# qiqiqicheng/news-recommendation-tc

Hardware: AMD Instinct MI355X
Metric: recalled pairs/sec (YouTubeDNN top-30) + DIN scored pairs/sec, 1/2/4/8 MI355X (higher is better)
Workload: dtype fp16

## Files before the change

### include/nrk.h

```cpp
#ifndef NRK_H
#define NRK_H

#include <stddef.h>
#include <stdint.h>

#ifdef __cplusplus
extern "C" {
#endif

typedef void* nrk_stream_t;

#define NRK_OK 0
#define NRK_EINVAL 1
#define NRK_EHIP 2
#define NRK_EUNSUPPORTED 3

const char* nrk_last_error(void);
#define NRK_ABI_VERSION 3
int nrk_abi_version(void);


int nrk_tt_user_fwd(const float* user_table, int64_t n_user_rows, const float* item_table,
                    int64_t n_item_rows, int dim, const int32_t* uid, const int32_t* hist,
                    const int32_t* hist_len, int64_t n, int seq_len, const float* w0,
                    const float* b0, int h0, const float* w1, const float* b1, int h1,
                    float* out, nrk_stream_t stream);

int nrk_tt_user_fwd_layers(const float* user_table, int64_t n_user_rows, const float* item_table,
                           int64_t n_item_rows, int dim, const int32_t* uid, const int32_t* hist,
                           const int32_t* hist_len, int64_t n, int seq_len, const float* weights, int n_layers,
                           const int* widths, float* out, nrk_stream_t stream);
int nrk_tt_item_fwd(const float* item_table, int64_t n_item_rows, int dim, const int32_t* ids,
                    int64_t n, float* out, nrk_stream_t stream);


size_t nrk_tt_train_workspace_bytes(int64_t n_user_rows, int64_t n_item_rows, int dim, int n_layers,
                                    const int* widths, int seq_len, int batch);

int nrk_tt_train_grad(const float* user_table, int64_t n_user_rows, const float* item_table,
                      int64_t n_item_rows, int dim, const float* weights, int n_layers, const int* widths,
                      const int64_t* log_off, const int32_t* log_items, const int32_t* s_user,
                      const int32_t* s_pos, const int32_t* s_target, const float* s_label, int batch,
                      int seq_len, float p, uint64_t seed, int64_t step, float* loss, float* w_grad,
                      int32_t* u_rows, float* u_vals, int32_t* u_count, int32_t* i_rows, float* i_vals,
                      int32_t* i_count, void* workspace, size_t workspace_bytes, nrk_stream_t stream);

int nrk_tt_dropout_mask(uint64_t seed, int64_t step, int layer, int batch, int width, float p, float* out,
                        nrk_stream_t stream);

int nrk_tt_adam_step(float* weights, float* w_m, float* w_v, const float* w_grad, int64_t n_weights,
                     float* user_table, float* u_m, float* u_v, int64_t n_user_rows, const int32_t* u_rows,
                     const float* u_vals, const int32_t* u_count, float* item_table, float* i_m, float* i_v,
                     int64_t n_item_rows, const int32_t* i_rows, const float* i_vals, const int32_t* i_count,
                     int dim, double lr, double beta1, double beta2, double eps, int64_t t,
                     nrk_stream_t stream);

int nrk_tt_make_samples_count(const int64_t* log_off, int64_t n_users, int64_t* pos_off, nrk_stream_t stream);
int nrk_tt_make_samples(const int64_t* log_off, const int32_t* log_items, int64_t n_users,
                        const int64_t* pos_off, int64_t n_pos, int negsample, const int32_t* pool,
                        int64_t n_pool, uint64_t seed, int32_t* s_user, int32_t* s_pos, int32_t* s_target,
                        float* s_label, nrk_stream_t stream);


size_t nrk_ip_catalog_bytes(int64_t n_items, int dim);
int nrk_ip_catalog_build(const float* items, int64_t n_items, int dim, void* catalog,
                         nrk_stream_t stream);

size_t nrk_ip_topk_workspace_bytes(int64_t n_users, int64_t n_items, int dim, int k);
int nrk_ip_topk(const float* users, int64_t n_users, const float* items, const void* catalog,
                int64_t n_items, int dim, int k, int64_t row_offset, float* out_scores,
                int32_t* out_rows, double* out_exact, void* workspace, size_t workspace_bytes,
                nrk_stream_t stream);

int nrk_ip_topk_screen(const float* users, int64_t n_users, const void* catalog, int64_t n_items,
                       int dim, int k, void* workspace, size_t workspace_bytes,
                       nrk_stream_t stream);
int nrk_ip_topk_scan(const float* users, int64_t n_users, const void* catalog, int64_t n_items, int dim, int k,
                     void* workspace, size_t workspace_bytes, nrk_stream_t stream);
int nrk_ip_topk_select(const float* users, int64_t n_users, const void* catalog, int64_t n_items, int dim, int k,
                       void* workspace, size_t workspace_bytes, nrk_stream_t stream);
int nrk_ip_topk_finish(const float* users, int64_t n_users, const float* items,
                       const void* catalog, int64_t n_items,
                       int dim, int k, int64_t row_offset, float* out_scores, int32_t* out_rows,
                       double* out_exact, void* workspace, size_t workspace_bytes,
                       nrk_stream_t stream);

int nrk_ip_topk_bound(const float* users, int64_t n_users, const void* catalog, int64_t n_items, int dim,
                      int k, int m, float* out_bound, void* workspace, size_t workspace_bytes,
                      nrk_stream_t stream);
int nrk_ip_topk_apply_bound(int64_t n_users, const float* bounds, int n_lists, int m, int k, void* workspace,
                            size_t workspace_bytes, nrk_stream_t stream);

int nrk_ip_topk_tile_blocks(int dim);

int nrk_ip_topk_shard_screen(const float* users, int64_t n_users, const void* catalog, int64_t n_items, int dim,
                             int k, int64_t blk_lo, int64_t blk_hi, int m, float* out_bound, void* workspace,
                             size_t workspace_bytes, nrk_stream_t stream);
int nrk_ip_topk_shard_band(int64_t n_users, int64_t n_items, int dim, int k, const float* bounds, int n_lists,
                           int m, int x_cap, void* workspace, size_t workspace_bytes, void* out_ent,
                           int32_t* out_cnt, nrk_stream_t stream);
int nrk_ip_topk_refine_x(const float* users, int64_t n_users, const float* items, const void* catalog,
                         int64_t n_items, int dim, int k, int64_t row_offset, const void* band, int n_src,
                         int64_t src_users, int x_cap, const int32_t* src_cnt, const float* ucut,
                         const int32_t* ovf_in, float* out_scores, int32_t* out_rows, double* out_exact,
                         void* workspace, size_t workspace_bytes, nrk_stream_t stream);

int nrk_topk_merge(const double* in_exact, const int32_t* in_rows, int n_lists,
                   int64_t list_stride, int64_t n_users, int k_in, int k_out, float* out_scores,
                   int32_t* out_rows, double* out_exact, nrk_stream_t stream);

#define NRK_IP_QUERY_MAX_USERS 4096
size_t nrk_ip_query_workspace_bytes(int64_t n_users, int64_t n_items, int dim, int k);
int nrk_ip_query_plan(int64_t n_users, int64_t n_items, int dim, int k, int32_t out[4]);
int nrk_ip_query(const float* users, int64_t n_users, const float* items, int64_t n_items, int dim, int k,
                 int64_t row_offset, float* out_scores, int32_t* out_rows, double* out_exact, void* workspace,
                 size_t workspace_bytes, nrk_stream_t stream);


int nrk_row_normalize(const float* x, int64_t n, int dim, float* out, float* norms,
                      nrk_stream_t stream);


int nrk_itemcf_pair_offsets(const int64_t* offsets, int64_t n_users, int64_t* pair_off,
                            nrk_stream_t stream);
size_t nrk_itemcf_workspace_bytes(int64_t n_pairs, int32_t n_items);
int nrk_itemcf_sim(const int64_t* offsets, int64_t n_users, const int32_t* items,
                   const int64_t* ts, const double* created, int32_t n_items,
                   const int64_t* pair_off, int64_t n_pairs, double loc_alpha,
                   double loc_alpha_rev, double loc_beta, double time_alpha,
                   double created_alpha, int32_t* out_i, int32_t* out_j, double* out_v,
                   int64_t* out_first, int64_t* out_n, int64_t* out_cnt, void* workspace,
                   size_t workspace_bytes, nrk_stream_t stream);

int nrk_itemcf_topn(const int64_t* row_off, int64_t n_rows, const int32_t* cols,
                    const double* vals, const int64_t* first, int topn, int32_t* out_cols,
                    double* out_vals, int32_t* out_cnt, nrk_stream_t stream);

int nrk_itemcf_pairs(const int64_t* offsets, int64_t n_users, const int32_t* items, const int64_t* ts,
                     const double* created, int32_t n_items, const int64_t* pair_off, int64_t slot_base,
                     double loc_alpha, double loc_alpha_rev, double loc_beta, double time_alpha,
                     double created_alpha, uint64_t* keys, int32_t* slots, double* w, int64_t* item_cnt,
                     nrk_stream_t stream);
size_t nrk_itemcf_reduce_workspace_bytes(int64_t n);
int nrk_itemcf_reduce(const uint64_t* keys, const int32_t* slots, const double* w, int64_t n, int32_t n_items,
                      const int64_t* item_cnt, int32_t* out_i, int32_t* out_j, double* out_v,
                      int64_t* out_first, int64_t* out_n, void* workspace, size_t workspace_bytes,
                      nrk_stream_t stream);

int nrk_itemcf_row_offsets(const int32_t* ei, int64_t n, int64_t n_rows, int64_t* row_off,
                           nrk_stream_t stream);

int nrk_itemcf_recall_offsets(const int64_t* q_slot, int64_t n_query, const int64_t* offsets,
                              const int32_t* items, const int32_t* nbr_cnt, int64_t* cand_off,
                              nrk_stream_t stream);
size_t nrk_itemcf_recall_workspace_bytes(int64_t n_cand);
int nrk_itemcf_recall(const int64_t* q_slot, int64_t n_query, const int64_t* offsets, const int32_t* items,
                      const int32_t* nbr_cols, const double* nbr_vals, const int32_t* nbr_cnt, int topn,
                      const double* created, int32_t n_items, const int32_t* hot, int n_hot,
                      const int32_t* emb_cols, const double* emb_vals, const int32_t* emb_cnt, int ke,
                      double loc_beta, double created_alpha, const int64_t* cand_off, int64_t n_cand,
                      int topk, int32_t* out_items, double* out_scores, int32_t* out_src,
                      int32_t* out_cnt, void* workspace, size_t workspace_bytes, nrk_stream_t stream);


size_t nrk_usercf_workspace_bytes(int64_t n_users, int64_t n_clicks, int topn);
int nrk_usercf_topn(const int64_t* i_off, int32_t n_items, const int32_t* i_users, const int64_t* u_off,
                    int64_t n_users, const int32_t* u_items, int64_t n_clicks, const double* act, const double* pen,
                    int topn, int32_t* out_cols, double* out_vals, int64_t* out_cnt, int32_t* out_nnz,
                    void* workspace, size_t workspace_bytes, nrk_stream_t stream);
int nrk_usercf_sim(const int64_t* i_off, int32_t n_items, const int32_t* i_users, const int64_t* u_off,
                   int64_t n_users, const int32_t* u_items, int64_t n_clicks, const double* act, const double* pen,
                   const int64_t* row_off, int64_t n_entries, int32_t* out_v, double* out_s, int64_t* out_first,
                   void* workspace, size_t workspace_bytes, nrk_stream_t stream);

int nrk_usercf_recall_offsets(const int64_t* q_slot, int64_t n_query, const int64_t* offsets,
                              const int32_t* nbr_cols, const int32_t* nbr_cnt, int topn, int64_t* cand_off,
                              nrk_stream_t stream);
size_t nrk_usercf_recall_workspace_bytes(int64_t n_cand);
int nrk_usercf_recall(const int64_t* q_slot, int64_t n_query, const int64_t* offsets, const int32_t* items,
// ... 184 lines not shown
```

### news-recommendation-tc_amd/csrc/tower.hip

```cpp
#include "tower_common.h"

namespace nrk {

template <int D>
__global__ __launch_bounds__(256) __attribute__((amdgpu_waves_per_eu(4))) void tt_user_kernel(
    const float* __restrict__ user_table, const float* __restrict__ item_table,
    const int32_t* __restrict__ uid, const int32_t* __restrict__ hist,
    const int32_t* __restrict__ hist_len, int64_t n, int T, const float* __restrict__ w0,
    const float* __restrict__ b0, int h0, const float* __restrict__ w1,
    const float* __restrict__ b1, int h1, float* __restrict__ out) {
    static_assert(D % 2 == 0 && D >= 16 && D <= 64 && (D & (D - 1)) == 0, "tt_user_kernel: D in {16, 32, 64}");
    extern __shared__ __attribute__((aligned(16))) float lds[];
    const int S0 = 2 * D + 4, h0p = (h0 + 3) & ~3, S1 = h0p + 4, h1p = (h1 + 3) & ~3;
    float* sw0 = lds;
    float* sb0 = sw0 + h0 * S0;
    float* sw1 = sb0 + h0p;
    float* sb1 = sw1 + h1 * S1;
    float* sx = sb1 + h1p + (threadIdx.x >> 6) * (2 * D + 128);
    for (int i = threadIdx.x; i < h0 * 2 * D; i += blockDim.x) sw0[(i / (2 * D)) * S0 + i % (2 * D)] = w0[i];
    for (int i = threadIdx.x; i < h0; i += blockDim.x) sb0[i] = b0[i];
    for (int i = threadIdx.x; i < h1 * h0; i += blockDim.x) sw1[(i / h0) * S1 + i % h0] = w1[i];
    for (int i = threadIdx.x; i < h1; i += blockDim.x) sb1[i] = b1[i];
    __syncthreads();

    constexpr int P = WAVE / D;
    constexpr int CH = 8;
    const int lane = threadIdx.x & 63, wave = threadIdx.x >> 6;
    const int d = lane % D, ph = lane / D;
    const int64_t wstride = (int64_t)gridDim.x * 4;
    auto meta = [&](int64_t uu, int& len, int32_t& uidv, int32_t& hv) {
        const bool ok = uu < n;
        len = ok ? hist_len[uu] : 0;
        uidv = ok ? uid[uu] : 0;
        hv = ok && lane < T ? hist[uu * T + lane] : 0;
    };
    int64_t u = (int64_t)blockIdx.x * 4 + wave;
    int len, uidv;
    int32_t hv;
    meta(u, len, uidv, hv);
    float pout = 0.0f;
    int64_t pu = -1;
    for (; u < n; u += wstride) {
        int nlen, nuid;
        int32_t nhv;
        meta(u + wstride, nlen, nuid, nhv);
        const float xu = user_table[(int64_t)uidv * D + d];
        float sum = 0.0f;
        const int nit = (len + P - 1) / P;
        for (int i0 = 0; i0 < nit; i0 += CH) {
            float v[CH];
#pragma unroll
            for (int e = 0; e < CH; ++e) {
                const int t = ph + P * (i0 + e);
                const int32_t r = __shfl(hv, t < T ? t : 0, WAVE);
                v[e] = item_table[(int64_t)(t < len ? r : 0) * D + d];
            }
            if (i0 == 0 && pu >= 0) {
                if (lane < h1) out[pu * h1 + lane] = pout;
                pu = -1;
            }
#pragma unroll
            for (int e = 0; e < CH; ++e)
                if (ph + P * (i0 + e) < len) sum += v[e];
        }
#pragma unroll
        for (int off = D; off < WAVE; off <<= 1) sum += __shfl_xor(sum, off, WAVE);
        const float xm = sum / ((float)len + 1e-8f);
        if (lane < D) {
            sx[lane] = xu;
            sx[D + lane] = xm;
        }
        __builtin_amdgcn_wave_barrier();
        float y0 = 0.0f, y1 = 0.0f;
        {
#pragma clang fp contract(off)
            float z0 = lane < h0 ? sb0[lane] : 0.0f;
            float z1 = lane + WAVE < h0 ? sb0[lane + WAVE] : 0.0f;
            const float* wr0 = sw0 + (lane < h0 ? lane : 0) * S0;
            const float* wr1 = sw0 + (lane + WAVE < h0 ? lane + WAVE : 0) * S0;
            if (h0 > WAVE) {
#pragma unroll 2
                for (int q = 0; q < 2 * D; q += 4) {
                    const float4 xq = *reinterpret_cast<const float4*>(sx + q);
                    const float4 a = *reinterpret_cast<const float4*>(wr0 + q);
                    const float4 b = *reinterpret_cast<const float4*>(wr1 + q);
                    z0 += a.x * xq.x;
                    z0 += a.y * xq.y;
                    z0 += a.z * xq.z;
                    z0 += a.w * xq.w;
                    z1 += b.x * xq.x;
                    z1 += b.y * xq.y;
                    z1 += b.z * xq.z;
                    z1 += b.w * xq.w;
                }
            } else {
#pragma unroll 2
                for (int q = 0; q < 2 * D; q += 4) {
                    const float4 xq = *reinterpret_cast<const float4*>(sx + q);
                    const float4 a = *reinterpret_cast<const float4*>(wr0 + q);
                    z0 += a.x * xq.x;
                    z0 += a.y * xq.y;
                    z0 += a.z * xq.z;
                    z0 += a.w * xq.w;
                }
            }
            y0 = fmaxf(z0, 0.0f);
            y1 = fmaxf(z1, 0.0f);
        }
        float* sy = sx + 2 * D;
        if (lane < h0) sy[lane] = y0;
        if (lane + WAVE < h0) sy[lane + WAVE] = y1;
        __builtin_amdgcn_wave_barrier();
        float v = 0.0f;
        {
#pragma clang fp contract(off)
            float z = lane < h1 ? sb1[lane] : 0.0f;
            const float* wr = sw1 + (lane < h1 ? lane : 0) * S1;
            int q = 0;
            for (; q + 4 <= h0; q += 4) {
                const float4 yq = *reinterpret_cast<const float4*>(sy + q);
                const float4 a = *reinterpret_cast<const float4*>(wr + q);
                z += a.x * yq.x;
                z += a.y * yq.y;
                z += a.z * yq.z;
                z += a.w * yq.w;
            }
            for (; q < h0; ++q) z += wr[q] * sy[q];
            v = lane < h1 ? fmaxf(z, 0.0f) : 0.0f;
        }
        __builtin_amdgcn_wave_barrier();
        const float nn = sqrtf(wave_sum_f32(v * v));
        v = v / fmaxf(nn, 1e-12f);
        float n2 = sqrtf(wave_sum_f32(v * v));
        if (n2 == 0.0f) n2 = 1.0f;
        if (pu >= 0 && lane < h1) out[pu * h1 + lane] = pout;
        pout = v / n2;
        pu = u;
        len = nlen;
        uidv = nuid;
        hv = nhv;
    }
    if (pu >= 0 && lane < h1) out[pu * h1 + lane] = pout;
}

template <int D>
__global__ __launch_bounds__(256) void tt_user_mlp_kernel(
    const float* __restrict__ user_table, const float* __restrict__ item_table,
    const int32_t* __restrict__ uid, const int32_t* __restrict__ hist,
    const int32_t* __restrict__ hist_len, int64_t n, int T, const float* __restrict__ wts, TtLayers ly,
    float* __restrict__ out) {
    __shared__ float sx[4][2][TT_MAXW > 2 * D ? TT_MAXW : 2 * D];
    const int lane = threadIdx.x & 63, wave = threadIdx.x >> 6;
    const int64_t wstride = (int64_t)gridDim.x * 4;
    for (int64_t u = (int64_t)blockIdx.x * 4 + wave; u < n; u += wstride) {
        const int32_t hv = lane < T ? hist[u * T + lane] : 0;
        const float xu = user_table[(int64_t)uid[u] * D + lane % D];
        const float xm = tt_hist_mean<D>(item_table, hv, hist_len[u], T, lane);
        if (lane < D) {
            sx[wave][0][lane] = xu;
            sx[wave][0][D + lane] = xm;
        }
        wave_sync_lds();
        int in = 2 * D, cur = 0;
        const float* wl = wts;
        for (int l = 0; l < ly.n; ++l) {
            const int wo = ly.w[l];
            const float* bl = wl + (size_t)wo * in;
            for (int o = lane; o < wo; o += WAVE) {
#pragma clang fp contract(off)
                float z = bl[o];
                const float* wr = wl + (size_t)o * in;
                for (int qq = 0; qq < in; ++qq) z += wr[qq] * sx[wave][cur][qq];
                sx[wave][cur ^ 1][o] = fmaxf(z, 0.0f);
            }
            wave_sync_lds();
            wl = bl + wo;
            in = wo;
            cur ^= 1;
        }
        const float v = lane < D ? sx[wave][cur][lane] : 0.0f;
        const float nn = sqrtf(wave_sum_f32(v * v));
        const float v1 = v / fmaxf(nn, 1e-12f);
        float n2 = sqrtf(wave_sum_f32(v1 * v1));
        if (n2 == 0.0f) n2 = 1.0f;
        if (lane < D) out[u * D + lane] = v1 / n2;
        wave_sync_lds();
    }
}

template <int D>
__global__ __launch_bounds__(256) void tt_item_kernel(const float* __restrict__ table,
                                                      const int32_t* __restrict__ ids, int64_t n,
                                                      float* __restrict__ out) {
    for (int64_t r = blockIdx.x * (int64_t)blockDim.x + threadIdx.x; r < n;
         r += (int64_t)gridDim.x * blockDim.x) {
        const float* src = table + (int64_t)ids[r] * D;
        float v[D];
        float s = 0.0f;
#pragma unroll
        for (int q = 0; q < D; ++q) {
            v[q] = src[q];
            s += v[q] * v[q];
        }
        const float inv = fmaxf(sqrtf(s), 1e-12f);
        float s2 = 0.0f;
#pragma unroll
        for (int q = 0; q < D; ++q) {
            v[q] = v[q] / inv;
            s2 += v[q] * v[q];
        }
        const float n2 = sqrtf(s2);
#pragma unroll
        for (int q = 0; q < D; ++q) out[r * D + q] = v[q] / n2;
    }
}

}

using namespace nrk;

static int tt_grid(const void* fn, size_t lds, int64_t n) {
    return (int)std::max<int64_t>(1, std::min<int64_t>((n + 3) / 4, resident_blocks(fn, 256, lds)));
}

constexpr size_t tt_user_lds(int dim, int h0, int h1) {
    const size_t h0p = (size_t)((h0 + 3) & ~3), h1p = (size_t)((h1 + 3) & ~3);
    return sizeof(float) *
           ((size_t)h0 * (2 * dim + 4) + h0p + (size_t)h1 * (h0p + 4) + h1p + (size_t)4 * (2 * dim + 128));
}
constexpr int TT_H0_MAX = 128;

extern "C" {

int nrk_tt_user_fwd(const float* user_table, int64_t n_user_rows, const float* item_table,
                    int64_t n_item_rows, int dim, const int32_t* uid, const int32_t* hist,
                    const int32_t* hist_len, int64_t n, int seq_len, const float* w0,
                    const float* b0, int h0, const float* w1, const float* b1, int h1,
                    float* out, nrk_stream_t stream) {
    clear_error();
    NRK_REQUIRE(n >= 0 && seq_len >= 1 && seq_len <= 64, "bad sizes (seq_len must be in [1, 64])");
    NRK_REQUIRE(n_user_rows > 0 && n_item_rows > 0, "empty embedding tables");
    if (const int rc = tt_check_shape(__func__, dim)) return rc;
    NRK_REQUIRE(h0 >= 1 && h0 <= TT_H0_MAX, "h0 must be in [1, 128]");
    NRK_REQUIRE(h1 == dim, TT_LAST_WIDTH);
    if (n == 0) return NRK_OK;
    NRK_REQUIRE(user_table && item_table && uid && hist && hist_len && w0 && b0 && w1 && b1 && out,
                "null pointer");
    const size_t lds = tt_user_lds(dim, h0, h1);
    hipStream_t s = as_stream(stream);
    tt_for_dim(dim, [&](auto dc) {
        constexpr int DD = decltype(dc)::value;
        constexpr size_t lds_max = tt_user_lds(DD, TT_H0_MAX, DD);
        static_assert(lds_max <= CU_LDS_BYTES, "tt_user_kernel LDS");
        static std::atomic<uint64_t> lds_set{0};
        lds_limit_once(lds_set, (const void*)tt_user_kernel<DD>, lds_max);
        const int grid = tt_grid((const void*)tt_user_kernel<DD>, lds, n);
        tt_user_kernel<DD><<<grid, 256, lds, s>>>(user_table, item_table, uid, hist, hist_len, n, seq_len, w0, b0, h0,
                                                  w1, b1, h1, out);
    });
    NRK_CHECK_LAUNCH();
    return NRK_OK;
}

int nrk_tt_user_fwd_layers(const float* user_table, int64_t n_user_rows, const float* item_table,
                           int64_t n_item_rows, int dim, const int32_t* uid, const int32_t* hist,
                           const int32_t* hist_len, int64_t n, int seq_len, const float* weights, int n_layers,
                           const int* widths, float* out, nrk_stream_t stream) {
    clear_error();
    NRK_REQUIRE(n >= 0 && seq_len >= 1 && seq_len <= 64, "bad sizes (seq_len must be in [1, 64])");
    NRK_REQUIRE(n_user_rows > 0 && n_item_rows > 0, "empty embedding tables");
    TtLayers ly{};
    if (const int rc = tt_check_shape(__func__, dim, n_layers, widths, &ly)) return rc;
    if (n == 0) return NRK_OK;
    NRK_REQUIRE(user_table && item_table && uid && hist && hist_len && weights && out, "null pointer");
    hipStream_t s = as_stream(stream);
    const unsigned grid = grid_for(n, 4, 2048);
    tt_for_dim(dim, [&](auto dc) {
        tt_user_mlp_kernel<decltype(dc)::value><<<grid, 256, 0, s>>>(user_table, item_table, uid, hist, hist_len, n,
                                                                     seq_len, weights, ly, out);
    });
    NRK_CHECK_LAUNCH();
    return NRK_OK;
}

int nrk_tt_item_fwd(const float* item_table, int64_t n_item_rows, int dim, const int32_t* ids,
                    int64_t n, float* out, nrk_stream_t stream) {
    clear_error();
    NRK_REQUIRE(n >= 0 && n_item_rows > 0, "bad sizes");
    if (const int rc = tt_check_shape(__func__, dim)) return rc;
    if (n == 0) return NRK_OK;
    NRK_REQUIRE(item_table && ids && out, "null pointer");
    hipStream_t s = as_stream(stream);
    const unsigned grid = grid_for(n, 256, 4096);
    tt_for_dim(dim, [&](auto dc) { tt_item_kernel<decltype(dc)::value><<<grid, 256, 0, s>>>(item_table, ids, n, out); });
    NRK_CHECK_LAUNCH();
    return NRK_OK;
}

}
```

### news-recommendation-tc_amd/nrk/_lib.py

```python
from __future__ import annotations

import ctypes
import os

_HERE = os.path.dirname(os.path.abspath(__file__))
LIB_PATH = os.environ.get("NRK_LIB_PATH") or os.path.join(_HERE, "libnrk.so")

NRK_OK, NRK_EINVAL, NRK_EHIP, NRK_EUNSUPPORTED = 0, 1, 2, 3

P = ctypes.c_void_p
I64 = ctypes.c_int64
I32 = ctypes.c_int32
INT = ctypes.c_int
F64 = ctypes.c_double
SZ = ctypes.c_size_t

SIGNATURES = {
    "nrk_last_error": (ctypes.c_char_p, []),
    "nrk_abi_version": (INT, []),
    "nrk_tt_user_fwd": (INT, [P, I64, P, I64, INT, P, P, P, I64, INT, P, P, INT, P, P, INT, P, P]),
    "nrk_tt_user_fwd_layers": (INT, [P, I64, P, I64, INT, P, P, P, I64, INT, P, INT, P, P, P]),
    "nrk_tt_item_fwd": (INT, [P, I64, INT, P, I64, P, P]),
    "nrk_tt_train_workspace_bytes": (SZ, [I64, I64, INT, INT, P, INT, INT]),
    "nrk_tt_train_grad": (INT, [P, I64, P, I64, INT, P, INT, P, P, P, P, P, P, P, INT, INT, ctypes.c_float,
                                ctypes.c_uint64, I64, P, P, P, P, P, P, P, P, P, SZ, P]),
    "nrk_tt_dropout_mask": (INT, [ctypes.c_uint64, I64, INT, INT, INT, ctypes.c_float, P, P]),
    "nrk_tt_adam_step": (INT, [P, P, P, P, I64, P, P, P, I64, P, P, P, P, P, P, I64, P, P, P, INT,
                               F64, F64, F64, F64, I64, P]),
    "nrk_tt_make_samples_count": (INT, [P, I64, P, P]),
    "nrk_tt_make_samples": (INT, [P, P, I64, P, I64, INT, P, I64, ctypes.c_uint64, P, P, P, P, P]),
    "nrk_ip_catalog_bytes": (SZ, [I64, INT]),
    "nrk_ip_catalog_build": (INT, [P, I64, INT, P, P]),
    "nrk_ip_topk_workspace_bytes": (SZ, [I64, I64, INT, INT]),
    "nrk_ip_topk_tile_blocks": (INT, [INT]),
    "nrk_ip_topk": (INT, [P, I64, P, P, I64, INT, INT, I64, P, P, P, P, SZ, P]),
    "nrk_ip_topk_screen": (INT, [P, I64, P, I64, INT, INT, P, SZ, P]),
    "nrk_ip_topk_finish": (INT, [P, I64, P, P, I64, INT, INT, I64, P, P, P, P, SZ, P]),
    "nrk_ip_topk_bound": (INT, [P, I64, P, I64, INT, INT, INT, P, P, SZ, P]),
    "nrk_ip_topk_apply_bound": (INT, [I64, P, INT, INT, INT, P, SZ, P]),
    "nrk_topk_merge": (INT, [P, P, INT, I64, I64, INT, INT, P, P, P, P]),
    "nrk_ip_topk_scan": (INT, [P, I64, P, I64, INT, INT, P, SZ, P]),
    "nrk_rccl_unique_id_bytes": (INT, []),
    "nrk_rccl_get_unique_id": (INT, [P]),
    "nrk_rccl_comm_init": (INT, [P, INT, P, INT]),
    "nrk_rccl_comm_destroy": (INT, [P]),
    "nrk_rccl_topk_allgather": (INT, [P, P, P, I64, INT, INT, P, P, P, P, P, P]),
    "nrk_rccl_bound_allgather": (INT, [P, P, I64, INT, P, P]),
    "nrk_rccl_band_alltoall": (INT, [P, P, P, I64, INT, P, P, P]),
    "nrk_ip_topk_select": (INT, [P, I64, P, I64, INT, INT, P, SZ, P]),
    "nrk_ip_topk_shard_screen": (INT, [P, I64, P, I64, INT, INT, I64, I64, INT, P, P, SZ, P]),
    "nrk_ip_topk_shard_band": (INT, [I64, I64, INT, INT, P, INT, INT, INT, P, SZ, P, P, P]),
    "nrk_ip_topk_refine_x": (INT, [P, I64, P, P, I64, INT, INT, I64, P, INT, I64, INT, P, P, P, P, P, P, P, SZ,
                                   P]),
    "nrk_ip_query_workspace_bytes": (SZ, [I64, I64, INT, INT]),
    "nrk_ip_query_plan": (INT, [I64, I64, INT, INT, P]),
    "nrk_ip_query": (INT, [P, I64, P, I64, INT, INT, I64, P, P, P, P, SZ, P]),
    "nrk_row_normalize": (INT, [P, I64, INT, P, P, P]),
    "nrk_itemcf_pair_offsets": (INT, [P, I64, P, P]),
    "nrk_itemcf_workspace_bytes": (SZ, [I64, I32]),
    "nrk_itemcf_sim": (INT, [P, I64, P, P, P, I32, P, I64, F64, F64, F64, F64, F64,
                             P, P, P, P, P, P, P, SZ, P]),
    "nrk_itemcf_topn": (INT, [P, I64, P, P, P, INT, P, P, P, P]),
    "nrk_itemcf_row_offsets": (INT, [P, I64, I64, P, P]),
    "nrk_itemcf_pairs": (INT, [P, I64, P, P, P, I32, P, I64, F64, F64, F64, F64, F64, P, P, P, P, P]),
    "nrk_itemcf_reduce_workspace_bytes": (SZ, [I64]),
    "nrk_itemcf_reduce": (INT, [P, P, P, I64, I32, P, P, P, P, P, P, P, SZ, P]),
    "nrk_itemcf_recall_offsets": (INT, [P, I64, P, P, P, P, P]),
    "nrk_itemcf_recall_workspace_bytes": (SZ, [I64]),
    "nrk_itemcf_recall": (INT, [P, I64, P, P, P, P, P, INT, P, I32, P, INT, P, P, P, INT, F64, F64, P, I64,
                                INT, P, P, P, P, P, SZ, P]),
    "nrk_usercf_workspace_bytes": (SZ, [I64, I64, INT]),
    "nrk_usercf_topn": (INT, [P, I32, P, P, I64, P, I64, P, P, INT, P, P, P, P, P, SZ, P]),
    "nrk_usercf_sim": (INT, [P, I32, P, P, I64, P, I64, P, P, P, I64, P, P, P, P, SZ, P]),
    "nrk_usercf_recall_offsets": (INT, [P, I64, P, P, P, INT, P, P]),
    "nrk_usercf_recall_workspace_bytes": (SZ, [I64]),
    "nrk_usercf_recall": (INT, [P, I64, P, P, P, P, P, INT, P, P, I32, P, INT, P, P, P, INT, F64, P, I64,
                                INT, P, P, P, P, P, SZ, P]),
    "nrk_din_assemble": (INT, [P, P, I64, INT, INT, INT, P, INT, P, I64, INT, P, P, INT, INT, INT,
                               ctypes.c_float, ctypes.c_float, ctypes.c_uint32, I64, I64, P, P, P, P, P, P, P]),
    "nrk_gather_rows": (INT, [P, I64, INT, P, I64, P, P]),
    "nrk_fuse_minmax": (INT, [P, I64, P, P]),
    "nrk_fuse": (INT, [P, I64, P, P, P, P, INT, P, INT, INT, F64, F64, P, P, P, P, INT, P, P, P, P]),
    "nrk_fuse_wide": (INT, [P, I64, P, P, P, P, INT, P, INT, INT, F64, F64, P, P, P, P, INT, INT, P, P, P, P]),
    "nrk_coldstart_filter": (INT, [P, I64, P, I64, P, P, P, I64, P, P, I64, P, P, P, P, I64, F64, F64, P, P, P]),
    "nrk_coldstart_recall": (INT, [P, I64, P, I64, P, P, I64, P, P, P, I64, P, P, I64, P, P, P, P, I64, F64, F64,
                                   INT, INT, P, P, P, P]),
    "nrk_profile_user": (INT, [P, I64, P, P, P, I64, INT, P, P, I64, P, P, P, P, P, P, P]),
    "nrk_profile_item_count": (INT, [P, I64, I64, P, P]),
    "nrk_profile_scale": (INT, [P, I64, P, INT, P, P]),
    "nrk_profile_labels": (INT, [P, P, I64, P, I64, INT, P, P]),
    "nrk_ctx_features": (INT, [P, P, P, P, P]),
    "nrk_ctx_fit_workspace_bytes": (SZ, [I64, I32]),
    "nrk_ctx_fit_tile": (I32, []),
    "nrk_ctx_fit_stats": (INT, [P, I64, I32, P, P, I32, P, I32, P, P, P, SZ, P]),
    "nrk_ctx_fit_count_below": (INT, [I64, I32, P, I32, P, P, SZ, P]),
    "nrk_din_remap_index": (INT, [P, I64, INT, P, INT, P, P]),
    "nrk_din_prep_bytes": (SZ, [INT, I64]),
    "nrk_din_prepare": (INT, [P, INT, P, INT, I64, P, P]),
    "nrk_din_workspace_bytes": (SZ, [I64, INT, INT, INT, INT, INT, INT]),
    "nrk_din_forward": (INT, [P, INT, P, INT, INT, INT, P, P, P, P, P, I64, INT, P, P, P, P,
                              P, P, INT, P, P, INT, P, P, P, P, P, SZ, P]),
    "nrk_din_segments_workspace_bytes": (SZ, [I64, I64, INT, INT, INT, INT, INT, INT]),
    "nrk_din_forward_segments": (INT, [P, INT, P, INT, INT, INT, P, P, P, P, P, I64, I64, INT, P, P,
                                       P, P, P, P, INT, P, P, INT, P, P, P, P, P, SZ, P]),
    "nrk_din_train_workspace_bytes": (SZ, [I64, INT, INT, INT, INT, INT, INT, INT, INT, I64, INT]),
    "nrk_din_train_grad": (INT, [P, I64, INT, INT, P, INT, INT, INT, P, INT, INT, INT, P, P, P, P, P, P, I64, INT,
                                 P, P, P, P, P, P, SZ, P]),
    "nrk_din_adam_step": (INT, [P, P, P, P, I64, P, P, P, I64, INT, P, P, P, F64, F64, F64, F64, I64, P]),
}

_lib = None


class NrkError(RuntimeError):
    pass


def lib():
    global _lib
    if _lib is None:
        if not os.path.exists(LIB_PATH):
            raise NrkError(
                f"libnrk.so not found at {LIB_PATH}; build it with "
                "`make -C news-recommendation-tc_amd` (or __graft_entry__.build())"
            )
        L = ctypes.CDLL(LIB_PATH)
        for name, (res, args) in SIGNATURES.items():
            fn = getattr(L, name, None)
            if fn is None:
                continue
            fn.restype = res
            fn.argtypes = args
        _lib = L
    return _lib


def exported_symbols():
    L = lib()
    return [n for n in SIGNATURES if getattr(L, n, None) is not None]


def check(rc: int, what: str = ""):
    if rc == NRK_OK:
        return
    msg = lib().nrk_last_error().decode(errors="replace")
    if rc == NRK_EINVAL:
        raise ValueError(f"{what}: {msg}")
    if rc == NRK_EUNSUPPORTED:
        raise NotImplementedError(f"{what}: {msg}")
    raise NrkError(f"{what}: {msg}")


def call(name: str, *args):
    rc = getattr(lib(), name)(*args)
    check(rc, name)
```

### news-recommendation-tc_amd/nrk/ops.py

```python
from __future__ import annotations

import torch

from . import _lib

_P = _lib.P


def _stream():
    return _P(torch.cuda.current_stream().cuda_stream)


def _ptr(t):
    return _P(t.data_ptr()) if t is not None else None


def _dev(*ts):
    dev = None
    for t in ts:
        if t is None:
            continue
        if not t.is_cuda:
            raise ValueError("nrk ops need device (cuda/HIP) tensors")
        if not t.is_contiguous():
            raise ValueError("nrk ops need contiguous tensors")
        if dev is None:
            dev = t.device
        elif t.device != dev:
            raise ValueError("tensors on different devices")
    return dev


def _need(t, dtype, shape=None, name="tensor"):
    if t.dtype != dtype:
        raise ValueError(f"{name}: expected {dtype}, got {t.dtype}")
    if shape is not None and tuple(t.shape) != tuple(shape):
        raise ValueError(f"{name}: expected shape {tuple(shape)}, got {tuple(t.shape)}")


def _finite(t, name):
    if t.numel() and not bool(torch.isfinite(t).all()):
        raise ValueError(f"{name} must be finite (NaN / inf found)")


def _tt_in_range(t, hi, what):
    if t.numel():
        lo_v, hi_v = torch.stack([t.min(), t.max()]).tolist()
        if lo_v < 0 or hi_v >= hi:
            raise ValueError(f"{what} out of [0, {hi})")


def tt_validate(uid, hist, hist_len, n_user_rows, n_item_rows):
    n, T = hist.shape
    if n == 0:
        return
    _tt_in_range(hist_len, T + 1, "hist_len")
    _tt_in_range(uid, int(n_user_rows), "uid")
    if T:
        live = torch.arange(T, device=hist.device)[None, :] < hist_len[:, None]
        _tt_in_range(torch.where(live, hist, torch.zeros((), dtype=hist.dtype, device=hist.device)),
                     int(n_item_rows), "live hist entry")


def tt_user_fwd(user_table, item_table, uid, hist, hist_len, w0, b0, w1, b1, validate: bool = True, out=None):
    _dev(user_table, item_table, uid, hist, hist_len, w0, b0, w1, b1)
    n, T = hist.shape
    D = user_table.shape[1]
    h0, h1 = w0.shape[0], w1.shape[0]
    _need(user_table, torch.float32, name="user_table")
    _need(item_table, torch.float32, (item_table.shape[0], D), "item_table")
    _need(uid, torch.int32, (n,), "uid")
    _need(hist, torch.int32, name="hist")
    _need(hist_len, torch.int32, (n,), "hist_len")
    _need(w0, torch.float32, (h0, 2 * D), "w0")
    _need(b0, torch.float32, (h0,), "b0")
    _need(w1, torch.float32, (h1, h0), "w1")
    _need(b1, torch.float32, (h1,), "b1")
    if validate:
        tt_validate(uid, hist, hist_len, user_table.shape[0], item_table.shape[0])
    if out is None:
        out = torch.empty((n, h1), dtype=torch.float32, device=uid.device)
    else:
        _dev(out)
        _need(out, torch.float32, (n, h1), "out")
        if not out.is_contiguous():
            raise ValueError("out must be contiguous")
    _lib.call("nrk_tt_user_fwd", _ptr(user_table), user_table.shape[0], _ptr(item_table),
              item_table.shape[0], D, _ptr(uid), _ptr(hist), _ptr(hist_len), n, T,
              _ptr(w0), _ptr(b0), h0, _ptr(w1), _ptr(b1), h1, _ptr(out), _stream())
    return out


def tt_user_fwd_layers(user_table, item_table, uid, hist, hist_len, layers):
    import ctypes

    _dev(user_table, item_table, uid, hist, hist_len, *[t for wb in layers for t in wb])
    n, T = hist.shape
    D = user_table.shape[1]
    _need(user_table, torch.float32, name="user_table")
    _need(item_table, torch.float32, (item_table.shape[0], D), "item_table")
    _need(uid, torch.int32, (n,), "uid")
    _need(hist, torch.int32, name="hist")
    _need(hist_len, torch.int32, (n,), "hist_len")
    widths, packed, fan_in = [], [], 2 * D
    for l, (w, b) in enumerate(layers):
        _need(w, torch.float32, (w.shape[0], fan_in), f"W{l}")
        _need(b, torch.float32, (w.shape[0],), f"b{l}")
        widths.append(int(w.shape[0]))
        packed += [w.reshape(-1), b]
        fan_in = w.shape[0]
    tt_validate(uid, hist, hist_len, user_table.shape[0], item_table.shape[0])
    wts = torch.cat(packed).contiguous()
    out = torch.empty((n, D), dtype=torch.float32, device=uid.device)
    wv = (ctypes.c_int * len(widths))(*widths)
    _lib.call("nrk_tt_user_fwd_layers", _ptr(user_table), user_table.shape[0], _ptr(item_table),
              item_table.shape[0], D, _ptr(uid), _ptr(hist), _ptr(hist_len), n, T, _ptr(wts), len(widths),
              ctypes.cast(wv, _P), _ptr(out), _stream())
    return out


def tt_item_fwd(item_table, ids, validate: bool = True):
    _dev(item_table, ids)
    _need(item_table, torch.float32, name="item_table")
    _need(ids, torch.int32, name="ids")
    n, D = ids.shape[0], item_table.shape[1]
    if validate:
        _tt_in_range(ids, item_table.shape[0], "ids")
    out = torch.empty((n, D), dtype=torch.float32, device=ids.device)
    _lib.call("nrk_tt_item_fwd", _ptr(item_table), item_table.shape[0], D, _ptr(ids), n,
              _ptr(out), _stream())
    return out


TT_MAX_BATCH = 8192
_tt_ws_cache = {}


def _tt_ws(dev, nbytes):
    ws = _tt_ws_cache.get(dev)
    if ws is None or ws.numel() < nbytes:
        ws = torch.empty(max(int(nbytes), 1), dtype=torch.uint8, device=dev)
        _tt_ws_cache[dev] = ws
    return ws


def tt_pack_layers(layers):
    return (torch.cat([t.reshape(-1) for wb in layers for t in wb]).contiguous(),
            [int(w.shape[0]) for w, _ in layers])


def tt_unpack_layers(weights, widths, dim):
    out, off, fan_in = [], 0, 2 * dim
    for w in widths:
        out.append((weights[off:off + w * fan_in].view(w, fan_in), weights[off + w * fan_in:off + w * fan_in + w]))
        off += w * fan_in + w
        fan_in = w
    return out


def _tt_n_weights(widths, dim):
    n, fan_in = 0, 2 * dim
    for w in widths:
        n += w * (fan_in + 1)
        fan_in = w
    return n


class TtGrads:

    def __init__(self, dev, batch, seq_len, dim, n_weights):
        f = dict(dtype=torch.float32, device=dev)
        i = dict(dtype=torch.int32, device=dev)
        self.batch, self.seq_len, self.dim = batch, seq_len, dim
        self.loss = torch.zeros(1, **f)
        self.w_grad = torch.empty(n_weights, **f)
        self.u_rows, self.u_vals, self.u_count = torch.empty(batch, **i), torch.empty((batch, dim), **f), torch.zeros(1, **i)
        cap = batch * (seq_len + 1)
        self.i_rows, self.i_vals, self.i_count = torch.empty(cap, **i), torch.empty((cap, dim), **f), torch.zeros(1, **i)

    def user_grad(self):
        n = int(self.u_count)
        return self.u_rows[:n], self.u_vals[:n]

    def item_grad(self):
        n = int(self.i_count)
        return self.i_rows[:n], self.i_vals[:n]


def tt_check_samples(n_user_rows, n_item_rows, log_off, log_items, s_user, s_pos, s_target, seq_len):
    if int(log_off[0]) != 0 or int(log_off[-1]) != log_items.shape[0] or bool((log_off[1:] < log_off[:-1]).any()):
        raise ValueError("log_off is not a CSR offset vector over log_items")
    if log_items.numel() and (int(log_items.min()) < 0 or int(log_items.max()) >= n_item_rows):
        raise ValueError("log_items out of [0, n_item_rows)")
    if not s_user.numel():
        return
    if int(s_user.min()) < 0 or int(s_user.max()) >= n_user_rows:
        raise ValueError("s_user out of [0, n_user_rows)")
    if int(s_target.min()) < 0 or int(s_target.max()) >= n_item_rows:
        raise ValueError("s_target out of [0, n_item_rows)")
    su = s_user.long()
    rowlen = log_off[su + 1] - log_off[su]
    if int(s_pos.min()) < 1 or bool((s_pos.long().clamp(max=seq_len) > rowlen).any()):
        raise ValueError("s_pos must be >= 1 and min(s_pos, seq_len) within the user's log row")


def tt_train_grad(user_table, item_table, weights, widths, log_off, log_items, s_user, s_pos, s_target, s_label,
                  seq_len, p: float = 0.0, seed: int = 0, step: int = 0, validate: bool = True, out=None, loss=None):
    import ctypes

    dev = _dev(user_table, item_table, weights, log_off, log_items, s_user, s_pos, s_target, s_label, loss)
    U, D = user_table.shape
    I = item_table.shape[0]
    B = s_user.shape[0]
    _need(user_table, torch.float32, name="user_table")
    _need(item_table, torch.float32, (I, D), "item_table")
    _need(weights, torch.float32, (_tt_n_weights(widths, D),), "weights")
    _need(log_off, torch.int64, (U + 1,), "log_off")
    _need(log_items, torch.int32, name="log_items")
    _need(s_user, torch.int32, (B,), "s_user")
    _need(s_pos, torch.int32, (B,), "s_pos")
    _need(s_target, torch.int32, (B,), "s_target")
    _need(s_label, torch.float32, (B,), "s_label")
    if loss is not None:
        _need(loss, torch.float32, (1,), "loss")
    if validate and B:
        tt_check_samples(U, I, log_off, log_items, s_user, s_pos, s_target, seq_len)
    wv = (ctypes.c_int * len(widths))(*widths)
    wp = ctypes.cast(wv, _P)
    nbytes = _lib.lib().nrk_tt_train_workspace_bytes(U, I, D, len(widths), wp, seq_len, B)
    if not nbytes:
        raise ValueError("nrk_tt_train_workspace_bytes: " + _lib.lib().nrk_last_error().decode(errors="replace"))
    ws = _tt_ws(dev, nbytes)
    if out is None:
        out = TtGrads(dev, B, seq_len, D, weights.numel())
    elif (out.batch, out.seq_len, out.dim, out.w_grad.numel()) != (B, seq_len, D, weights.numel()):
        raise ValueError("out: a TtGrads of another shape")
    _lib.call("nrk_tt_train_grad", _ptr(user_table), U, _ptr(item_table), I, D, _ptr(weights), len(widths), wp,
              _ptr(log_off), _ptr(log_items), _ptr(s_user), _ptr(s_pos), _ptr(s_target), _ptr(s_label), B,
              seq_len, float(p), int(seed) & (2 ** 64 - 1), int(step), _ptr(out.loss if loss is None else loss),
              _ptr(out.w_grad), _ptr(out.u_rows), _ptr(out.u_vals), _ptr(out.u_count), _ptr(out.i_rows),
              _ptr(out.i_vals), _ptr(out.i_count), _ptr(ws), ws.numel(), _stream())
    return out

# ... 1110 lines not shown
```

Baseline: 1.323 billion.

## Batch four users per wave in the two-tower user forward kernel

Adds a new user-tower kernel in which each wave processes a group of four users together. The history gather spreads lanes across users and dims, and the two MLP layers run as small vectorised matmuls, so each LDS weight load is reused across four users instead of one. It is dispatched whenever h0 is at most the wave size, and a query function reports the group size. The cost is more registers and LDS per wave and new, fairly intricate index and reduction logic that risks correctness bugs at the edges.

```diff
diff --git a/include/nrk.h b/include/nrk.h
--- a/include/nrk.h
+++ b/include/nrk.h
@@ -25,6 +25,8 @@
                     const int32_t* hist_len, int64_t n, int seq_len, const float* w0,
                     const float* b0, int h0, const float* w1, const float* b1, int h1,
                     float* out, nrk_stream_t stream);
+
+int nrk_tt_user_pass_users(int dim, int h0);
 
 int nrk_tt_user_fwd_layers(const float* user_table, int64_t n_user_rows, const float* item_table,
                            int64_t n_item_rows, int dim, const int32_t* uid, const int32_t* hist,
diff --git a/news-recommendation-tc_amd/csrc/tower.hip b/news-recommendation-tc_amd/csrc/tower.hip
--- a/news-recommendation-tc_amd/csrc/tower.hip
+++ b/news-recommendation-tc_amd/csrc/tower.hip
@@ -143,6 +143,204 @@
     if (pu >= 0 && lane < h1) out[pu * h1 + lane] = pout;
 }
 
+constexpr int TT_PASS_G = 4;
+constexpr int tt_pass_tile(int dim) { return 2 * dim * TT_PASS_G + 64 * TT_PASS_G; }
+template <int N>
+using fvec = float __attribute__((ext_vector_type(N)));
+typedef fvec<2> f32x2;
+typedef fvec<4> f32x4;
+
+template <int D>
+__global__ __launch_bounds__(256) __attribute__((amdgpu_waves_per_eu(4))) void tt_user_kernel_pass(
+    const float* __restrict__ user_table, const float* __restrict__ item_table,
+    const int32_t* __restrict__ uid, const int32_t* __restrict__ hist,
+    const int32_t* __restrict__ hist_len, int64_t n, int T, const float* __restrict__ w0,
+    const float* __restrict__ b0, int h0, const float* __restrict__ w1,
+    const float* __restrict__ b1, float* __restrict__ out) {
+    static_assert(D == 16 || D == 32 || D == 64, "tt_user_kernel_pass: D in {16, 32, 64}");
+    constexpr int G = TT_PASS_G, h1 = D;
+    constexpr int P = WAVE / D;
+    constexpr int UL = G * D / WAVE;
+    extern __shared__ __attribute__((aligned(16))) float lds[];
+    const int S0 = 2 * D + 4, h0p = (h0 + 3) & ~3, S1 = h0p + 4;
+    float* sw0 = lds;
+    float* sb0 = sw0 + h0 * S0;
+    float* sw1 = sb0 + h0p;
+    float* sb1 = sw1 + h1 * S1;
+    const int lane = threadIdx.x & 63, wave = __builtin_amdgcn_readfirstlane(threadIdx.x >> 6);
+    float* xs = sb1 + h1 + wave * tt_pass_tile(D);
+    float* ys = xs + 2 * D * G;
+    for (int i = threadIdx.x; i < h0 * 2 * D; i += blockDim.x) sw0[(i / (2 * D)) * S0 + i % (2 * D)] = w0[i];
+    for (int i = threadIdx.x; i < h0; i += blockDim.x) sb0[i] = b0[i];
+    for (int i = threadIdx.x; i < h1 * h0; i += blockDim.x) sw1[(i / h0) * S1 + i % h0] = w1[i];
+    for (int i = threadIdx.x; i < h1; i += blockDim.x) sb1[i] = b1[i];
+    __syncthreads();
+
+    constexpr int CH = 4;
+    const int d = lane % D, ph = lane / D;
+    const int64_t npass = (n + G - 1) / G, pstride = (int64_t)__builtin_amdgcn_readfirstlane(gridDim.x) * 4;
+    auto meta = [&](int64_t pp, int (&len)[G], int32_t (&uidv)[G], int32_t (&hv)[G]) {
+#pragma unroll
+        for (int g = 0; g < G; ++g) {
+            const int64_t uu = pp * G + g;
+            const bool ok = uu < n;
+            len[g] = ok ? hist_len[uu] : 0;
+            uidv[g] = ok ? uid[uu] : 0;
+            hv[g] = ok && lane < T ? hist[uu * T + lane] : 0;
+        }
+    };
+    int64_t p = (int64_t)blockIdx.x * 4 + wave;
+    int len[G];
+    int32_t uidv[G], hv[G];
+    meta(p, len, uidv, hv);
+    float pout[UL] = {};
+    int64_t prev = -1;
+    auto store_rows = [&]() {
+        const int64_t r0 = prev * G + UL * ph;
+#pragma unroll
+        for (int j = 0; j < UL; ++j)
+            if (r0 + j < n) out[(r0 + j) * h1 + d] = pout[j];
+        prev = -1;
+    };
+    for (; p < npass; p += pstride) {
+        int nlen[G];
+        int32_t nuid[G], nhv[G];
+        meta(p + pstride, nlen, nuid, nhv);
+        float xu[G], sum[G];
+        int nit[G], nl[G], nitmax = 0;
+#pragma unroll
+        for (int g = 0; g < G; ++g) {
+            xu[g] = user_table[(int64_t)uidv[g] * D + d];
+            ys[g * 64 + (lane % P) * D + lane / P] = __int_as_float(hv[g]);
+            sum[g] = 0.0f;
+            const int ln = len[g] < T ? len[g] : T;
+            nit[g] = (ln + P - 1) / P;
+            nl[g] = (ln + P - 1 - ph) / P;
+            nitmax = nit[g] > nitmax ? nit[g] : nitmax;
+        }
+        wave_sync_lds();
+        for (int i0 = 0; i0 < nitmax; i0 += CH) {
+            float v[G][CH];
+#pragma unroll
+            for (int g = 0; g < G; ++g) {
+                if (i0 < nit[g]) {
+                    const f32x4 r4 = *reinterpret_cast<const f32x4*>(ys + g * 64 + ph * D + i0);
+#pragma unroll
+                    for (int e = 0; e < CH; ++e) {
+                        const uint32_t r = i0 + e < nl[g] ? (uint32_t)__float_as_int(r4[e]) : 0u;
+                        v[g][e] = item_table[(int64_t)r * D + d];
+                    }
+                }
+            }
+            if (i0 == 0 && prev >= 0) store_rows();
+#pragma unroll
+            for (int g = 0; g < G; ++g) {
+                if (i0 < nit[g]) {
+#pragma unroll
+                    for (int e = 0; e < CH; ++e)
+                        if (i0 + e < nl[g]) sum[g] += v[g][e];
+                }
+            }
+        }
+        f32x4 xu4, xm4;
+#pragma unroll
+        for (int g = 0; g < G; ++g) {
+#pragma unroll
+            for (int off = D; off < WAVE; off <<= 1) sum[g] += __shfl_xor(sum[g], off, WAVE);
+            xu4[g] = xu[g];
+            xm4[g] = sum[g] / ((float)len[g] + 1e-8f);
+        }
+        wave_sync_lds();
+        if (lane < D) {
+            *reinterpret_cast<f32x4*>(xs + lane * G) = xu4;
+            *reinterpret_cast<f32x4*>(xs + (D + lane) * G) = xm4;
+        }
+        wave_sync_lds();
+        {
+#pragma clang fp contract(off)
+            const int o = lane < h0 ? lane : 0;
+            const float* wr0 = sw0 + o * S0;
+            const float bz = lane < h0 ? sb0[lane] : 0.0f;
+            f32x2 z01 = {bz, bz}, z23 = {bz, bz};
+#pragma unroll 2
+            for (int q = 0; q < 2 * D; q += 4) {
+                const f32x4 a = *reinterpret_cast<const f32x4*>(wr0 + q);
+#pragma unroll
+                for (int j = 0; j < 4; ++j) {
+                    const f32x4 x = *reinterpret_cast<const f32x4*>(xs + (q + j) * G);
+                    const f32x2 w = {a[j], a[j]};
+                    z01 = z01 + w * x.xy;
+                    z23 = z23 + w * x.zw;
+                }
+            }
+            if (lane < h0) {
+                const f32x4 y = {fmaxf(z01.x, 0.0f), fmaxf(z01.y, 0.0f), fmaxf(z23.x, 0.0f), fmaxf(z23.y, 0.0f)};
+                if constexpr (UL == 4) {
+                    *reinterpret_cast<f32x4*>(ys + lane * 4) = y;
+                } else if constexpr (UL == 2) {
+                    *reinterpret_cast<f32x2*>(ys + lane * 2) = y.xy;
+                    *reinterpret_cast<f32x2*>(ys + 128 + lane * 2) = y.zw;
+                } else {
+#pragma unroll
+                    for (int g = 0; g < G; ++g) ys[g * 64 + lane] = y[g];
+                }
+            }
+            wave_sync_lds();
+            const float* wr = sw1 + d * S1;
+            const float* yp = ys + ph * (64 * UL);
+            fvec<UL> z = (fvec<UL>)(sb1[d]);
+            int q = 0;
+            for (; q + 4 <= h0; q += 4) {
+                const f32x4 a = *reinterpret_cast<const f32x4*>(wr + q);
+                float yb[4 * UL];
+#pragma unroll
+                for (int k = 0; k < UL; ++k) {
+                    const f32x4 t = *reinterpret_cast<const f32x4*>(yp + q * UL + 4 * k);
+#pragma unroll
+                    for (int j = 0; j < 4; ++j) yb[4 * k + j] = t[j];
+                }
+#pragma unroll
+                for (int j = 0; j < 4; ++j) {
+                    fvec<UL> y;
+#pragma unroll
+                    for (int k = 0; k < UL; ++k) y[k] = yb[j * UL + k];
+                    z = z + (fvec<UL>)(a[j]) * y;
+                }
+            }
+            for (; q < h0; ++q) z = z + (fvec<UL>)(wr[q]) * *reinterpret_cast<const fvec<UL>*>(yp + q * UL);
+            float v[UL], nrm[UL];
+#pragma unroll
+            for (int j = 0; j < UL; ++j) v[j] = fmaxf(z[j], 0.0f);
+            wave_sync_lds();
+            auto norms = [&]() {
+#pragma unroll
+                for (int j = 0; j < UL; ++j) {
+                    float s = v[j] * v[j];
+                    if constexpr (D == WAVE) s = __builtin_fmaf(v[j], v[j], __shfl_xor(s, 32, WAVE));
+#pragma unroll
+                    for (int m = (D == WAVE ? 16 : D / 2); m > 0; m >>= 1) s = s + __shfl_xor(s, m, WAVE);
+                    nrm[j] = sqrtf(s);
+                }
+            };
+            norms();
+#pragma unroll
+            for (int j = 0; j < UL; ++j) v[j] = v[j] / fmaxf(nrm[j], 1e-12f);
+            norms();
+            if (prev >= 0) store_rows();
+#pragma unroll
+            for (int j = 0; j < UL; ++j) pout[j] = v[j] / (nrm[j] == 0.0f ? 1.0f : nrm[j]);
+        }
+        prev = p;
+#pragma unroll
+        for (int g = 0; g < G; ++g) {
+            len[g] = nlen[g];
+            uidv[g] = nuid[g];
+            hv[g] = nhv[g];
+        }
+    }
+    if (prev >= 0) store_rows();
+}
+
 template <int D>
 __global__ __launch_bounds__(256) void tt_user_mlp_kernel(
     const float* __restrict__ user_table, const float* __restrict__ item_table,
@@ -230,6 +428,13 @@
 }
 constexpr int TT_H0_MAX = 128;
 
+constexpr size_t tt_pass_lds(int dim, int h0) {
+    const size_t h0p = (size_t)((h0 + 3) & ~3);
+    return sizeof(float) * ((size_t)h0 * (2 * dim + 4) + h0p + (size_t)dim * (h0p + 4) + dim +
+                            (size_t)4 * tt_pass_tile(dim));
+}
+static int tt_pass_users(int h0) { return h0 <= WAVE ? TT_PASS_G : 0; }
+
 extern "C" {
 
 int nrk_tt_user_fwd(const float* user_table, int64_t n_user_rows, const float* item_table,
@@ -248,6 +453,20 @@
                 "null pointer");
     const size_t lds = tt_user_lds(dim, h0, h1);
     hipStream_t s = as_stream(stream);
+    if (tt_pass_users(h0)) {
+        const size_t plds = tt_pass_lds(dim, h0);
+        const int64_t want = (n + 4 * TT_PASS_G - 1) / (4 * TT_PASS_G);
+        tt_for_dim(dim, [&](auto dc) {
+            constexpr int DD = decltype(dc)::value;
+            static_assert(tt_pass_lds(DD, WAVE) <= 65536, "tt_user_kernel_pass LDS: under the default limit");
+            const int grid = (int)std::max<int64_t>(
+                1, std::min(want, resident_blocks((const void*)tt_user_kernel_pass<DD>, 256, plds)));
+            tt_user_kernel_pass<DD><<<grid, 256, plds, s>>>(user_table, item_table, uid, hist, hist_len, n, seq_len, w0,
+                                                            b0, h0, w1, b1, out);
+        });
+        NRK_CHECK_LAUNCH();
+        return NRK_OK;
+    }
     tt_for_dim(dim, [&](auto dc) {
         constexpr int DD = decltype(dc)::value;
         constexpr size_t lds_max = tt_user_lds(DD, TT_H0_MAX, DD);
@@ -260,6 +479,16 @@
     });
     NRK_CHECK_LAUNCH();
     return NRK_OK;
+}
+
+int nrk_tt_user_pass_users(int dim, int h0) {
+    clear_error();
+    if (tt_check_shape(__func__, dim)) return 0;
+    if (h0 < 1 || h0 > TT_H0_MAX) {
+        fail_as(__func__, NRK_EINVAL, "h0 must be in [1, 128]");
+        return 0;
+    }
+    return tt_pass_users(h0);
 }
 
 int nrk_tt_user_fwd_layers(const float* user_table, int64_t n_user_rows, const float* item_table,
diff --git a/news-recommendation-tc_amd/nrk/_lib.py b/news-recommendation-tc_amd/nrk/_lib.py
--- a/news-recommendation-tc_amd/nrk/_lib.py
+++ b/news-recommendation-tc_amd/nrk/_lib.py
@@ -19,6 +19,7 @@
     "nrk_last_error": (ctypes.c_char_p, []),
     "nrk_abi_version": (INT, []),
     "nrk_tt_user_fwd": (INT, [P, I64, P, I64, INT, P, P, P, I64, INT, P, P, INT, P, P, INT, P, P]),
+    "nrk_tt_user_pass_users": (INT, [INT, INT]),
     "nrk_tt_user_fwd_layers": (INT, [P, I64, P, I64, INT, P, P, P, I64, INT, P, INT, P, P, P]),
     "nrk_tt_item_fwd": (INT, [P, I64, INT, P, I64, P, P]),
     "nrk_tt_train_workspace_bytes": (SZ, [I64, I64, INT, INT, P, INT, INT]),
diff --git a/news-recommendation-tc_amd/nrk/ops.py b/news-recommendation-tc_amd/nrk/ops.py
--- a/news-recommendation-tc_amd/nrk/ops.py
+++ b/news-recommendation-tc_amd/nrk/ops.py
@@ -89,6 +89,14 @@
               item_table.shape[0], D, _ptr(uid), _ptr(hist), _ptr(hist_len), n, T,
               _ptr(w0), _ptr(b0), h0, _ptr(w1), _ptr(b1), h1, _ptr(out), _stream())
     return out
+
+
+def tt_user_pass_users(d: int, h0: int) -> int:
+    L = _lib.lib()
+    g = L.nrk_tt_user_pass_users(int(d), int(h0))
+    if g == 0 and L.nrk_last_error():
+        raise ValueError(L.nrk_last_error().decode(errors="replace"))
+    return g
 
 
 def tt_user_fwd_layers(user_table, item_table, uid, hist, hist_len, layers):
```

New measurement: 1.347 billion, median of 6. +1.9%, better.
